# MinJunKang/DualPixelFace

Hardware: AMD Instinct MI355X
Metric: train samples/sec, StereoDPNet 1024x1536 DP pair (higher is better)
Workload: dtype f32

## Files before the change

### dualpixelface_amd/csrc/dcn_lean.hip

```cpp
#include "dcn_internal.h"
#include "conv_internal.h"

namespace {

typedef float f32x2 __attribute__((ext_vector_type(2)));

struct LeanP {
  int B, C, K, D, H, W;
  int Cpad, KT;
  long long P;
  int tilesY, tilesX;
  int nchunk;
};

__device__ __forceinline__ int lean_xcd_tile(int blk, int n) {
  const int q = n >> 3, r = n & 7, x = blk & 7, i = blk >> 3;
  return x * q + (x < r ? x : r) + i;
}

template <int CH_, int TY_, int TX_, int RYH_, int RXL_, int RXR_>
struct Geo {
  static constexpr int CH = CH_, NQ = CH_ / 4, TY = TY_, TX = TX_, RYH = RYH_, RXL = RXL_;
  static constexpr int NV = 4 * TY * TX;
  static constexpr int RY = TY + 2 + 2 * RYH;
  static constexpr int RX = (TX + 2 + RXL + RXR_ + 3) / 4 * 4;
  static constexpr int ZS = RY * RX * 16;
  static constexpr int PLANE = 4 * ZS;
  static constexpr int SQ = NV * 16;
  static constexpr int SBUF = NQ * SQ;
  static constexpr int LDS = NQ * PLANE + 2 * SBUF;
  static constexpr int NS = NV / 64;
  static_assert((1 + RXL) % 4 == 0 && TX % 16 == 0 && NV % 64 == 0, "aligned region origin / whole waves");
};

__device__ __forceinline__ int lane_pos32(int l) { return (int)((0x73261540u >> (4 * (l >> 2))) & 7u) * 4 + (l & 3); }

__device__ __forceinline__ f32x2 pk_mul_lo(f32x2 w, f32x2 v) {
  f32x2 r;
  asm("v_pk_mul_f32 %0, %1, %2 op_sel_hi:[0,1]" : "=v"(r) : "v"(w), "v"(v));
  return r;
}
__device__ __forceinline__ f32x2 pk_mul_hi(f32x2 w, f32x2 v) {
  f32x2 r;
  asm("v_pk_mul_f32 %0, %1, %2 op_sel:[1,0] op_sel_hi:[1,1]" : "=v"(r) : "v"(w), "v"(v));
  return r;
}
__device__ __forceinline__ void pk_fma_lo(f32x2& acc, f32x2 w, f32x2 v) {
  asm("v_pk_fma_f32 %0, %1, %2, %0 op_sel_hi:[0,1,1]" : "+v"(acc) : "v"(w), "v"(v));
}
__device__ __forceinline__ void pk_fma_hi(f32x2& acc, f32x2 w, f32x2 v) {
  asm("v_pk_fma_f32 %0, %1, %2, %0 op_sel:[1,0,0] op_sel_hi:[1,1,1]" : "+v"(acc) : "v"(w), "v"(v));
}

template <class G>
__device__ __forceinline__ void lean_stage(const LeanP& p, const float* __restrict__ xb, int c0, char* region, int ry0, int rx0, int tid,
                                           int nthreads) {
  constexpr int SR = G::RX / 4;
  const long long chan = p.P;
  const int units = p.D * G::RY * G::NQ * SR;
  for (int u = tid; u < units; u += nthreads) {
    const int seg = u % SR;
    const int it = u / SR;
    const int cg = it % G::NQ;
    const int row = it / G::NQ;
    const int lz = row / G::RY, ly = row - lz * G::RY;
    const int gy = ry0 + ly, gx = rx0 + 4 * seg;
    const bool ok = gy >= 0 && gy < p.H && gx >= 0 && gx < p.W;
    const float* src = xb + (long long)(c0 + 4 * cg) * chan + ((long long)lz * p.H + gy) * p.W + gx;
    f32x4 v[4];
#pragma unroll
    for (int q = 0; q < 4; ++q) v[q] = (ok && c0 + 4 * cg + q < p.C) ? *reinterpret_cast<const f32x4*>(src + q * chan) : f32x4{0.f, 0.f, 0.f, 0.f};
    char* dst = region + cg * G::PLANE + (row * G::RX + 4 * seg) * 16;
    *reinterpret_cast<f32x4*>(dst) = f32x4{v[0].x, v[1].x, v[2].x, v[3].x};
    *reinterpret_cast<f32x4*>(dst + 16) = f32x4{v[0].y, v[1].y, v[2].y, v[3].y};
    *reinterpret_cast<f32x4*>(dst + 32) = f32x4{v[0].z, v[1].z, v[2].z, v[3].z};
    *reinterpret_cast<f32x4*>(dst + 48) = f32x4{v[0].w, v[1].w, v[2].w, v[3].w};
  }
}

struct LeanTab {
  int a0, a1;
  f32x2 w00, w01, w10, w11;
  int d0, h0, w0;
  float ld, lh, lw;
  bool inreg;
  bool slow;
  f32x2 wz, wy, wx;
  f32x2 mz;
};

template <class G>
__device__ __forceinline__ LeanTab lean_tab(const LeanP& p, bool pvalid, int ry0, int rx0, float fd, float fh, float fw) {
  LeanTab t;
  const float d0f = floorf(fd), h0f = floorf(fh), w0f = floorf(fw);
  t.ld = fd - d0f; t.lh = fh - h0f; t.lw = fw - w0f;
  t.d0 = (int)d0f; t.h0 = (int)h0f; t.w0 = (int)w0f;
  const int ly = t.h0 - ry0, lx = t.w0 - rx0;
  t.inreg = (unsigned)ly < (unsigned)(G::RY - 1) && (unsigned)lx < (unsigned)(G::RX - 1);
  const bool valid = pvalid && fd > -1.f && fh > -1.f && fw > -1.f && fd < (float)p.D && fh < (float)p.H && fw < (float)p.W;
  const bool ok = t.inreg && valid;
  t.slow = valid && !t.inreg;
  const bool mz0 = (unsigned)t.d0 < (unsigned)p.D, mz1 = (unsigned)(t.d0 + 1) < (unsigned)p.D;
  f32x2 wz, wy, wx;
  wz.x = (ok && mz0) ? 1.f - t.ld : 0.f;
  wz.y = (ok && mz1) ? t.ld : 0.f;
  wy.x = 1.f - t.lh; wy.y = t.lh;
  wx.x = 1.f - t.lw; wx.y = t.lw;
  t.wz = wz; t.wy = wy; t.wx = wx;
  t.mz.x = (ok && mz0) ? 1.f : 0.f; t.mz.y = (ok && mz1) ? 1.f : 0.f;
  const int Dm1 = p.D - 1;
  const int iz0 = min(max(t.d0, 0), Dm1), iz1 = min(max(t.d0 + 1, 0), Dm1);
  const int cell = ok ? __mul24(__mul24(iz0, G::RY) + ly, G::RX) + lx : 0;
  t.a0 = cell * 16;
  t.a1 = t.a0 + __mul24(iz1 - iz0, G::ZS);
  const f32x2 zy0 = pk_mul_lo(wz, wy), zy1 = pk_mul_hi(wz, wy);
  t.w00 = pk_mul_lo(zy0, wx); t.w01 = pk_mul_hi(zy0, wx);
  t.w10 = pk_mul_lo(zy1, wx); t.w11 = pk_mul_hi(zy1, wx);
  return t;
}

#define LEAN_LOAD8(dst, q)                                                                        \
  dst[0] = *reinterpret_cast<const f32x4*>(r0 + (q) * G::PLANE);                                  \
  dst[1] = *reinterpret_cast<const f32x4*>(r0 + (q) * G::PLANE + 16);                             \
  dst[2] = *reinterpret_cast<const f32x4*>(r0 + (q) * G::PLANE + G::RX * 16);                     \
  dst[3] = *reinterpret_cast<const f32x4*>(r0 + (q) * G::PLANE + G::RX * 16 + 16);                \
  dst[4] = *reinterpret_cast<const f32x4*>(r1 + (q) * G::PLANE);                                  \
  dst[5] = *reinterpret_cast<const f32x4*>(r1 + (q) * G::PLANE + 16);                             \
  dst[6] = *reinterpret_cast<const f32x4*>(r1 + (q) * G::PLANE + G::RX * 16);                     \
  dst[7] = *reinterpret_cast<const f32x4*>(r1 + (q) * G::PLANE + G::RX * 16 + 16);

template <int CH>
__global__ void lean_repack_fwd1_kernel(const float* __restrict__ w, float* __restrict__ wl, int K, int C, int MT, int nchunk) {
  const int total = 27 * nchunk * MT * 512;
  for (int i = blockIdx.x * blockDim.x + threadIdx.x; i < total; i += gridDim.x * blockDim.x) {
    const int s = i & 7, lane = (i >> 3) & 63;
    int r = i >> 9;
    const int m = r % MT; r /= MT;
    const int chunk = r % nchunk;
    const int t = r / nchunk;
    const int k = 32 * m + (lane & 31), cl = 2 * s + (lane >> 5), c = chunk * CH + cl;
    wl[i] = (cl < CH && k < K && c < C) ? w[((long long)k * C + c) * 27 + t] : 0.f;
  }
}

template <class G, int MT>
__global__ __launch_bounds__(256, 2) void dcn_lean_fwd1_kernel(const float* __restrict__ x, const float* __restrict__ offset,
                                                            const float* __restrict__ wl, const float* __restrict__ bias,
                                                            float* __restrict__ out, LeanP p) {
  extern __shared__ __align__(16) char smem[];
  constexpr int CH = G::CH, NQ = G::NQ, KSTEPS = CH / 2, T = 27;
  static_assert(G::NV == 256, "four waves of 64 voxels");
  char* region = smem;
  const int tid = threadIdx.x, lane = tid & 63, l31 = lane & 31, hh = lane >> 5;
  const int wave_u = __builtin_amdgcn_readfirstlane(tid >> 6);
  int blk = lean_xcd_tile(blockIdx.x, gridDim.x);
  const int tx = blk % p.tilesX; blk /= p.tilesX;
  const int ty = blk % p.tilesY;
  const int b = blk / p.tilesY;
  const int y0 = ty * G::TY, x0 = tx * G::TX;
// ... 371 lines not shown
    tab1 = lean_tab<G>(p, pvalid, ry0, rx0, fd1, fh1, fw1);
  }
  int chunk = 0;
#pragma unroll 1
  for (int c0 = 0; c0 < p.C; c0 += CH, ++chunk) {
    __syncthreads();
    lean_stage<G>(p, xb, c0, region, ry0, rx0, tid, 256);
    load_a(0, chunk, aC);
    __syncthreads();
    sample_core();
    slow_fix(tab, nxt, c0);
    make_b(nxt, bH, bM, bL);
    tab = tab1;
#pragma unroll 1
    for (int t = 0; t < T - 1; ++t) {
      load_a(t + 1, chunk, aN);
      __builtin_amdgcn_sched_barrier(0);
      mfmas();
      sample_core();
      int u = t + 2;
      if (u >= T) u -= T;
      const LeanTab tabn = next_table(u);
#pragma unroll
      for (int i = 0; i < 4 * MT; ++i) {
        __builtin_amdgcn_sched_group_barrier(0x008, 1, 0);
        __builtin_amdgcn_sched_group_barrier(0x100, MT == 2 ? 2 : 4, 0);
        __builtin_amdgcn_sched_group_barrier(0x002, MT == 2 ? 2 : 4, 0);
      }
#pragma unroll
      for (int i = 0; i < 8 * MT; ++i) {
        __builtin_amdgcn_sched_group_barrier(0x008, 1, 0);
        __builtin_amdgcn_sched_group_barrier(0x002, MT == 2 ? 9 : 18, 0);
        __builtin_amdgcn_sched_group_barrier(0x100, MT == 2 ? 1 : 2, 0);
      }
      __builtin_amdgcn_sched_barrier(0);
      slow_fix(tab, nxt, c0);
      tab = tabn;
      make_b(nxt, bH, bM, bL);
#pragma unroll
      for (int m = 0; m < MT; ++m)
#pragma unroll
        for (int c = 0; c < 3; ++c) aC[m][c] = aN[m][c];
    }
    mfmas();
    tab1 = next_table(1);
  }
#pragma unroll
  for (int nt = 0; nt < 2; ++nt) {
    const int vo = wave_u * 64 + nt * 32 + lane_pos32(l31);
    const int qx = vo % G::TX, qy = (vo / G::TX) % G::TY, qz = vo / (G::TX * G::TY);
    const int gz = qz, gy = y0 + qy, gx = x0 + qx;
    const int q = l31 & 3;
    const bool o1 = (q & 1) != 0, o2 = (q & 2) != 0;
    const bool inb = gz < p.D && gy < p.H && gx < p.W;
    const long long pos = ((long long)gz * p.H + gy) * p.W + (gx - q);
#pragma unroll
    for (int m = 0; m < MT; ++m)
#pragma unroll
      for (int i = 0; i < 4; ++i) {
        float r0 = acc[m][nt][4 * i], r1 = acc[m][nt][4 * i + 1], r2 = acc[m][nt][4 * i + 2], r3 = acc[m][nt][4 * i + 3];
        {
          const float xa = o1 ? r0 : r1, ya = o1 ? r2 : r3;
          const float xs = __builtin_bit_cast(float, __builtin_amdgcn_mov_dpp(__builtin_bit_cast(int, xa), 0xB1, 0xf, 0xf, true));
          const float ys = __builtin_bit_cast(float, __builtin_amdgcn_mov_dpp(__builtin_bit_cast(int, ya), 0xB1, 0xf, 0xf, true));
          if (o1) { r0 = xs; r2 = ys; } else { r1 = xs; r3 = ys; }
        }
        {
          const float xa = o2 ? r0 : r2, ya = o2 ? r1 : r3;
          const float xs = __builtin_bit_cast(float, __builtin_amdgcn_mov_dpp(__builtin_bit_cast(int, xa), 0x4E, 0xf, 0xf, true));
          const float ys = __builtin_bit_cast(float, __builtin_amdgcn_mov_dpp(__builtin_bit_cast(int, ya), 0x4E, 0xf, 0xf, true));
          if (o2) { r0 = xs; r1 = ys; } else { r2 = xs; r3 = ys; }
        }
        const int k = m * 32 + 8 * i + 4 * hh + q;
        if (inb && k < p.K) {
          const float bv = bias ? bias[k] : 0.f;
          const f32x4 v = {r0 + bv, r1 + bv, r2 + bv, r3 + bv};
          *reinterpret_cast<f32x4*>(out + ((long long)b * p.K + k) * p.P + pos) = v;
        }
      }
  }
}

constexpr int LEAN_SS = 260;
constexpr int LEAN_NREP = DCN_WG_NREP;

template <class G>
struct BwdLds {
  static constexpr int GT = G::NQ * G::SQ;
  static constexpr int ST = G::CH * LEAN_SS * 4;
  static constexpr int OFF_G = G::NQ * G::PLANE;
  static constexpr int OFF_S = OFF_G + 2 * GT;
  static constexpr int LDS = OFF_S + 2 * ST;
  static_assert(G::NV == 256, "4 sampler waves + 4 matrix waves of 64 voxels");
};

typedef _Float16 lean_f16x8 __attribute__((ext_vector_type(8)));
typedef unsigned lean_u32x4 __attribute__((ext_vector_type(4)));
template <class G, bool GH>
__global__ __launch_bounds__(512) void dcn_lean_bwd_offset_kernel(const float* __restrict__ x, const float* __restrict__ offset,
                                                                  const float* __restrict__ wg ,
                                                                  const float* __restrict__ go, float* __restrict__ doff, float* __restrict__ dwtmp,
                                                                  LeanP p, int det) {
  extern __shared__ __align__(16) char smem[];
  constexpr int CH = G::CH, NQ = G::NQ, T = 27;
  typedef BwdLds<G> L;
  char* region = smem;
  const int tid = threadIdx.x, lane = tid & 63;
  const int wave_u = __builtin_amdgcn_readfirstlane(tid >> 6);
  int blk = lean_xcd_tile(blockIdx.x, gridDim.x);
  const int tx = blk % p.tilesX; blk /= p.tilesX;
  const int ty = blk % p.tilesY;
  const int b = blk / p.tilesY;
  const int y0 = ty * G::TY, x0 = tx * G::TX;
  const int ry0 = y0 - 1 - G::RYH, rx0 = x0 - 1 - G::RXL;
  const float* xb = x + (long long)b * p.C * p.P;
  const float* gob = go + (long long)b * p.K * p.P;
  const int NS = p.nchunk * T;
  if (wave_u < 4) {
    const int vox = wave_u * 64 + (lane & 32) + lane_pos32(lane & 31);
    const int px = vox % G::TX, py = (vox / G::TX) % G::TY, pz = vox / (G::TX * G::TY);
    const int zo = pz, yo = y0 + py, xo = x0 + px;
    const bool pvalid = zo < p.D && yo < p.H && xo < p.W;
    const long long ppos = pvalid ? ((long long)zo * p.H + yo) * p.W + xo : 0;
    const float* offp0 = offset + (long long)b * 3 * T * p.P + ppos;
    float* doffp0 = doff + (long long)b * 3 * T * p.P + ppos;
    const float zbf = (float)(zo - 1), ybf = (float)(yo - 1), xbf = (float)(xo - 1);
    const long long P3 = 3 * p.P;
    float od[3], oh[3], ow[3];
    LeanTab tab = lean_tab<G>(p, pvalid, ry0, rx0, zbf + offp0[0], ybf + offp0[p.P], xbf + offp0[2 * p.P]);
#pragma unroll
    for (int u = 1; u <= 3; ++u) { od[u % 3] = offp0[u * P3]; oh[u % 3] = offp0[u * P3 + p.P]; ow[u % 3] = offp0[u * P3 + 2 * p.P]; }
    lean_stage<G>(p, xb, 0, region, ry0, rx0, tid, 512);
    __syncthreads();
    int i = 0;
#pragma unroll 1
    for (int c0 = 0; c0 < p.C; c0 += CH) {
      if (c0 > 0) {
        lean_stage<G>(p, xb, c0, region, ry0, rx0, tid, 512);
        __syncthreads();
      }
#pragma unroll 1
      for (int g = 0; g < 9; ++g) {
        const int gn = g < 8 ? g + 1 : 0;
        const int ti = g / 3, tj = g - 3 * ti, tin = gn / 3, tjn = gn - 3 * tin;
        const float fz_same = zbf + (float)ti, fy_same = ybf + (float)tj, fz_next = zbf + (float)tin, fy_next = ybf + (float)tjn;
#pragma unroll
        for (int r = 0; r < 3; ++r, ++i) {
          const int t = 3 * g + r;
          const int sl = (r + 1) % 3;
          const float fdn = (r < 2 ? fz_same : fz_next) + od[sl], fhn = (r < 2 ? fy_same : fy_next) + oh[sl];
          const float fwn = (xbf + (float)((r + 1) % 3)) + ow[sl];
          {
            int u = t + 4;
            if (u >= T) u -= T;
            const float* np = offp0 + (long long)u * P3;
            od[sl] = np[0]; oh[sl] = np[p.P]; ow[sl] = np[2 * p.P];
          }
          const char* gt = smem + L::OFF_G + (i & 1) * L::GT + vox * 16;
          float* st = reinterpret_cast<float*>(smem + L::OFF_S + (i & 1) * L::ST);
          const char* r0 = region + tab.a0;
          const char* r1 = region + tab.a1;
          const f32x2 w00 = pk_mul_lo(pk_mul_lo(tab.wz, tab.wy), tab.wx), w01 = pk_mul_hi(pk_mul_lo(tab.wz, tab.wy), tab.wx);
          const f32x2 w10 = pk_mul_lo(pk_mul_hi(tab.wz, tab.wy), tab.wx), w11 = pk_mul_hi(pk_mul_hi(tab.wz, tab.wy), tab.wx);
          f32x4 cr[2][8], gq[2];
          LEAN_LOAD8(cr[0], 0)
          gq[0] = *reinterpret_cast<const f32x4*>(gt);
          LeanTab tabn = lean_tab<G>(p, pvalid, ry0, rx0, fdn, fhn, fwn);
          f32x2 dot[8];
#pragma unroll
          for (int q = 0; q < NQ; ++q) {
            if (q + 1 < NQ) {
              LEAN_LOAD8(cr[(q + 1) & 1], q + 1)
              gq[(q + 1) & 1] = *reinterpret_cast<const f32x4*>(gt + (q + 1) * G::SQ);
            }
            const f32x4* c = cr[q & 1];
            const f32x2 glo = gq[q & 1].xy, ghi = gq[q & 1].zw;
            f32x2 lo = pk_mul_lo(w00, c[0].xy), hi = pk_mul_lo(w00, c[0].zw);
            pk_fma_hi(lo, w00, c[1].xy); pk_fma_hi(hi, w00, c[1].zw);
            pk_fma_lo(lo, w01, c[2].xy); pk_fma_lo(hi, w01, c[2].zw);
            pk_fma_hi(lo, w01, c[3].xy); pk_fma_hi(hi, w01, c[3].zw);
            pk_fma_lo(lo, w10, c[4].xy); pk_fma_lo(hi, w10, c[4].zw);
            pk_fma_hi(lo, w10, c[5].xy); pk_fma_hi(hi, w10, c[5].zw);
            pk_fma_lo(lo, w11, c[6].xy); pk_fma_lo(hi, w11, c[6].zw);
            pk_fma_hi(lo, w11, c[7].xy); pk_fma_hi(hi, w11, c[7].zw);
            st[(4 * q + 0) * LEAN_SS + vox] = lo.x; st[(4 * q + 1) * LEAN_SS + vox] = lo.y;
            st[(4 * q + 2) * LEAN_SS + vox] = hi.x; st[(4 * q + 3) * LEAN_SS + vox] = hi.y;
#pragma unroll
            for (int j = 0; j < 8; ++j) {
              if (q == 0) dot[j] = glo * c[j].xy; else dot[j] = __builtin_elementwise_fma(glo, c[j].xy, dot[j]);
              dot[j] = __builtin_elementwise_fma(ghi, c[j].zw, dot[j]);
            }
          }
          float gd, gh, gw;
          {
            float d[8];
#pragma unroll
            for (int j = 0; j < 8; ++j) d[j] = dot[j].x + dot[j].y;
            const float wx0 = tab.wx.x, wx1 = tab.wx.y, wy0 = tab.wy.x, wy1 = tab.wy.y, wz0 = tab.wz.x, wz1 = tab.wz.y;
            const float A00 = fmaf(wx1, d[1], wx0 * d[0]), A01 = fmaf(wx1, d[3], wx0 * d[2]);
            const float A10 = fmaf(wx1, d[5], wx0 * d[4]), A11 = fmaf(wx1, d[7], wx0 * d[6]);
            const float E00 = fmaf(wy1, d[2], wy0 * d[0]), E01 = fmaf(wy1, d[3], wy0 * d[1]);
            const float E10 = fmaf(wy1, d[6], wy0 * d[4]), E11 = fmaf(wy1, d[7], wy0 * d[5]);
            const float B0 = fmaf(wy1, A01, wy0 * A00), B1 = fmaf(wy1, A11, wy0 * A10);
            gd = fmaf(tab.mz.y, B1, -tab.mz.x * B0);
            gh = fmaf(wz1, A11 - A10, wz0 * (A01 - A00));
            gw = fmaf(wz1, E11 - E10, wz0 * (E01 - E00));
          }
          unsigned long long slow = __ballot(tab.slow);
          while (slow) {
            const int Lq = __builtin_ctzll(slow);
            slow &= slow - 1;
            const int sd0 = __builtin_amdgcn_readlane(tab.d0, Lq), sh0 = __builtin_amdgcn_readlane(tab.h0, Lq), sw0 = __builtin_amdgcn_readlane(tab.w0, Lq);
            const float sld = __builtin_bit_cast(float, __builtin_amdgcn_readlane(__builtin_bit_cast(int, tab.ld), Lq));
            const float slh = __builtin_bit_cast(float, __builtin_amdgcn_readlane(__builtin_bit_cast(int, tab.lh), Lq));
            const float slw = __builtin_bit_cast(float, __builtin_amdgcn_readlane(__builtin_bit_cast(int, tab.lw), Lq));
            const int svox = __builtin_amdgcn_readlane(vox, Lq);
            const int ch = lane & 15, jd = lane >> 5, jh = (lane >> 4) & 1;
            const int dz = sd0 + jd, hy = sh0 + jh;
            const int cgl = c0 + ch;
            const bool rowin = ch < CH && cgl < p.C && (unsigned)dz < (unsigned)p.D && (unsigned)hy < (unsigned)p.H;
            const bool in0 = rowin && (unsigned)sw0 < (unsigned)p.W, in1 = rowin && (unsigned)(sw0 + 1) < (unsigned)p.W;
            const float* xr = xb + (long long)(cgl < p.C ? cgl : 0) * p.P + ((long long)(rowin ? dz : 0) * p.H + (rowin ? hy : 0)) * p.W;
            const float v0 = in0 ? xr[sw0] : 0.f, v1 = in1 ? xr[sw0 + 1] : 0.f;
            const float gch = ch < CH ? *reinterpret_cast<const float*>(smem + L::OFF_G + (i & 1) * L::GT + (ch >> 2) * G::SQ + svox * 16 + (ch & 3) * 4) : 0.f;
            const float wzj = jd ? sld : 1.f - sld, wyj = jh ? slh : 1.f - slh;
            float part = (wzj * wyj) * fmaf(slw, v1, (1.f - slw) * v0);
            part += __shfl_xor(part, 16, 64);
            part += __shfl_xor(part, 32, 64);
            if (lane < CH) st[lane * LEAN_SS + svox] = part;
            float e0 = gch * v0, e1 = gch * v1;
#pragma unroll
            for (int m = 1; m < 16; m <<= 1) { e0 += __shfl_xor(e0, m, 64); e1 += __shfl_xor(e1, m, 64); }
            const float ex = fmaf(slw, e1, (1.f - slw) * e0);
            float sgd = (jd ? 1.f : -1.f) * wyj * ex;
            float sgh = (jh ? 1.f : -1.f) * wzj * ex;
            float sgw = wzj * wyj * (e1 - e0);
            sgd += __shfl_xor(sgd, 16, 64); sgd += __shfl_xor(sgd, 32, 64);
            sgh += __shfl_xor(sgh, 16, 64); sgh += __shfl_xor(sgh, 32, 64);
            sgw += __shfl_xor(sgw, 16, 64); sgw += __shfl_xor(sgw, 32, 64);
            if (lane == Lq) { gd = sgd; gh = sgh; gw = sgw; }
          }
          if (pvalid) {
            float* dq = doffp0 + (long long)(3 * t) * p.P;
            if (c0 == 0) { dq[0] = gd; dq[p.P] = gh; dq[2 * p.P] = gw; }
            else { atomicAdd(dq, gd); atomicAdd(dq + p.P, gh); atomicAdd(dq + 2 * p.P, gw); }
          }
          tab = tabn;
          __syncthreads();
        }
      }
    }
  } else {
    const int mw = wave_u - 4, l15 = lane & 15, lg = lane >> 4;
    float bfrag[GH ? 1 : 4][16];
    lean_u32x4 bq[GH ? 4 : 1][2][2];
    int Egv[GH ? 4 : 1], Ew = DPF_H3_EMIN;
    if constexpr (GH) {
      Ew = __builtin_amdgcn_readfirstlane(reinterpret_cast<const int*>(wg)[27 * p.nchunk * 1024]);
#pragma unroll
      for (int s4 = 0; s4 < 4; ++s4) {
        const int vox = mw * 64 + s4 * 16 + l15;
        const int px = vox % G::TX, py = (vox / G::TX) % G::TY, pz = vox / (G::TX * G::TY);
        const bool ok = pz < p.D && y0 + py < p.H && x0 + px < p.W;
        const long long gpos = ok ? ((long long)pz * p.H + y0 + py) * p.W + x0 + px : 0;
        float gv[16];
        float mxg = 0.f;
#pragma unroll
        for (int mf = 0; mf < 2; ++mf)
#pragma unroll
          for (int i = 0; i < 8; ++i) {
            const int k = 32 * mf + 8 * lg + i;
            gv[8 * mf + i] = (ok && k < p.K) ? gob[(long long)k * p.P + gpos] : 0.f;
            mxg = __builtin_fmaxf(mxg, __builtin_fabsf(gv[8 * mf + i]));
          }
        mxg = __builtin_fmaxf(mxg, __shfl_xor(mxg, 16, 64));
        mxg = __builtin_fmaxf(mxg, __shfl_xor(mxg, 32, 64));
        int e = (int)(__builtin_bit_cast(unsigned, mxg) >> 23);
        e = e < DPF_H3_EMIN ? DPF_H3_EMIN : (e > 254 ? 254 : e);
        Egv[s4] = e;
        const float scg = dpf_h3_scale(e);
#pragma unroll
        for (int mf = 0; mf < 2; ++mf)
#pragma unroll
          for (int i = 0; i < 4; ++i) {
            unsigned h, l;
            dpf_split_pair_h(gv[8 * mf + 2 * i] * scg, gv[8 * mf + 2 * i + 1] * scg, h, l);
            bq[s4][mf][0][i] = h; bq[s4][mf][1][i] = l;
          }
      }
    } else {
#pragma unroll
      for (int s4 = 0; s4 < 4; ++s4) {
        const int vox = mw * 64 + s4 * 16 + l15;
        const int px = vox % G::TX, py = (vox / G::TX) % G::TY, pz = vox / (G::TX * G::TY);
        const bool ok = pz < p.D && y0 + py < p.H && x0 + px < p.W;
        const long long gpos = ok ? ((long long)pz * p.H + y0 + py) * p.W + x0 + px : 0;
#pragma unroll
        for (int ks = 0; ks < 16; ++ks) {
          const int k = 4 * ks + lg;
          bfrag[s4][ks] = (ok && k < p.K) ? gob[(long long)k * p.P + gpos] : 0.f;
        }
      }
    }
    float wfrag[64];
    {
      const int kk = 16 * mw + l15;
#pragma unroll
      for (int ks = 0; ks < 64; ++ks) {
        const int vox = 16 * (ks >> 2) + 4 * lg + (ks & 3);
        const int px = vox % G::TX, py = (vox / G::TX) % G::TY, pz = vox / (G::TX * G::TY);
        const bool ok = kk < p.K && pz < p.D && y0 + py < p.H && x0 + px < p.W;
        wfrag[ks] = ok ? gob[(long long)kk * p.P + ((long long)pz * p.H + y0 + py) * p.W + x0 + px] : 0.f;
      }
    }
    float* rep = det ? dwtmp : dwtmp + (long long)(blockIdx.x % LEAN_NREP) * T * p.nchunk * 64 * 16;
    long long* rep_shadow = det ? reinterpret_cast<long long*>(dwtmp) : nullptr;
    const int brow = (l15 < CH ? l15 : CH - 1) * LEAN_SS + 4 * lg;
    const unsigned wlane = (unsigned)lane * 64u;
    auto gcol = [&](int j) {
      const int chunk = j / T, t = j - chunk * T;
      const char* wb = reinterpret_cast<const char*>(wg) + (long long)(t * p.nchunk + chunk) * 4096;
      char* dst = smem + L::OFF_G + (j & 1) * L::GT + lg * G::SQ + (mw * 64 + l15) * 16;
      f32x4 a4[4];
      lean_u32x4 aq[2][2];
      if constexpr (GH) {
#pragma unroll
        for (int u = 0; u < 4; ++u) aq[u >> 1][u & 1] = *reinterpret_cast<const lean_u32x4*>(wb + u * 1024 + lane * 16);
      } else {
#pragma unroll
        for (int u = 0; u < 4; ++u) a4[u] = *reinterpret_cast<const f32x4*>(wb + wlane + 16 * u);
      }
#pragma unroll
      for (int sp2 = 0; sp2 < 2; ++sp2) {
        f32x4 acc[2] = {f32x4{0.f, 0.f, 0.f, 0.f}, f32x4{0.f, 0.f, 0.f, 0.f}};
        if constexpr (GH) {
          constexpr int ca[3] = {1, 0, 0}, cb[3] = {0, 1, 0};
#pragma unroll
          for (int i = 0; i < 3; ++i)
#pragma unroll
            for (int mf = 0; mf < 2; ++mf)
#pragma unroll
              for (int u = 0; u < 2; ++u)
                acc[u] = __builtin_amdgcn_mfma_f32_16x16x32_f16(__builtin_bit_cast(lean_f16x8, aq[mf][ca[i]]),
                                                                 __builtin_bit_cast(lean_f16x8, bq[2 * sp2 + u][mf][cb[i]]), acc[u], 0, 0, 0);
#pragma unroll
          for (int u = 0; u < 2; ++u)
#pragma unroll
            for (int r = 0; r < 4; ++r) acc[u][r] = __builtin_ldexpf(acc[u][r], Egv[2 * sp2 + u] + Ew - 282);
        } else {
#pragma unroll
          for (int ks = 0; ks < 16; ++ks)
#pragma unroll
            for (int u = 0; u < 2; ++u) acc[u] = __builtin_amdgcn_mfma_f32_16x16x4f32(a4[ks >> 2][ks & 3], bfrag[2 * sp2 + u][ks], acc[u], 0, 0, 0);
        }
        if (lg < NQ) {
          *reinterpret_cast<f32x4*>(dst + (2 * sp2) * 256) = acc[0];
          *reinterpret_cast<f32x4*>(dst + (2 * sp2 + 1) * 256) = acc[1];
        }
      }
    };
    gcol(0);
    lean_stage<G>(p, xb, 0, region, ry0, rx0, tid, 512);
    __syncthreads();
#pragma unroll 1
    for (int i = 0; i <= NS; ++i) {
      if (i + 1 < NS) gcol(i + 1);
      if (i >= 1) {
        const int j = i - 1, cs = j / T, ts = j - cs * T;
        const float* src = reinterpret_cast<const float*>(smem + L::OFF_S + (j & 1) * L::ST) + brow;
        f32x4 wacc[4] = {f32x4{0.f, 0.f, 0.f, 0.f}, f32x4{0.f, 0.f, 0.f, 0.f}, f32x4{0.f, 0.f, 0.f, 0.f}, f32x4{0.f, 0.f, 0.f, 0.f}};
#pragma unroll
        for (int qq = 0; qq < 16; ++qq) {
          const f32x4 bv = *reinterpret_cast<const f32x4*>(src + 16 * qq);
          wacc[0] = __builtin_amdgcn_mfma_f32_16x16x4f32(wfrag[4 * qq + 0], bv.x, wacc[0], 0, 0, 0);
          wacc[1] = __builtin_amdgcn_mfma_f32_16x16x4f32(wfrag[4 * qq + 1], bv.y, wacc[1], 0, 0, 0);
          wacc[2] = __builtin_amdgcn_mfma_f32_16x16x4f32(wfrag[4 * qq + 2], bv.z, wacc[2], 0, 0, 0);
          wacc[3] = __builtin_amdgcn_mfma_f32_16x16x4f32(wfrag[4 * qq + 3], bv.w, wacc[3], 0, 0, 0);
        }
        if (l15 < CH && cs * CH + l15 < p.C) {
          float* dst = rep + ((long long)(ts * p.nchunk + cs) * 64 + 16 * mw + 4 * lg) * 16 + l15;
#pragma unroll
          for (int r = 0; r < 4; ++r)
            if (16 * mw + 4 * lg + r < p.K) dcn_acc_add(rep, rep_shadow, &dst[r * 16], (wacc[0][r] + wacc[1][r]) + (wacc[2][r] + wacc[3][r]));
        }
      }
      if (i < NS) {
        __syncthreads();
        if (i + 1 < NS && (i + 1) % T == 0) {
          lean_stage<G>(p, xb, ((i + 1) / T) * CH, region, ry0, rx0, tid, 512);
          __syncthreads();
        }
      }
    }
  }
}

__global__ void lean_repack_gcol_kernel(const float* __restrict__ w, float* __restrict__ wg, int K, int C, int CH, int nchunk) {
  const int total = 27 * nchunk * 1024;
  for (int i = blockIdx.x * blockDim.x + threadIdx.x; i < total; i += gridDim.x * blockDim.x) {
    const int ks = i & 15, lane = (i >> 4) & 63;
    const int r = i >> 10;
    const int chunk = r % nchunk, t = r / nchunk;
    const int k = 4 * ks + (lane >> 4), l15 = lane & 15, c = chunk * CH + l15;
    wg[i] = (k < K && l15 < CH && c < C) ? w[((long long)k * C + c) * 27 + t] : 0.f;
  }
}

__global__ void lean_repack_gcol_h_kernel(const float* __restrict__ w, unsigned short* __restrict__ wgh, int K, int C, int CH, int nchunk) {
  __shared__ int s_e[16];
  float m = 0.f;
  const int nw = K * C * 27;
  for (int i = threadIdx.x; i < nw; i += blockDim.x) m = __builtin_fmaxf(m, __builtin_fabsf(w[i]));
  const int e = dpf_wave_max_exp(__builtin_bit_cast(unsigned, m));
  if ((threadIdx.x & 63) == 0) s_e[threadIdx.x >> 6] = e;
  __syncthreads();
  int E = DPF_H3_EMIN;
  for (int i = 0; i < (int)(blockDim.x >> 6); ++i) E = s_e[i] > E ? s_e[i] : E;
  E = E > 254 ? 254 : E;
  const float sc = dpf_h3_scale(E);
  const int total = 27 * nchunk * 2048;
  if (blockIdx.x == 0 && threadIdx.x == 0) reinterpret_cast<int*>(wgh)[total / 2] = E;
  for (int i = blockIdx.x * blockDim.x + threadIdx.x; i < total; i += gridDim.x * blockDim.x) {
    const int idx = i & 7, lane = (i >> 3) & 63, comp = (i >> 9) & 1, mf = (i >> 10) & 1;
    const int r = i >> 11;
    const int chunk = r % nchunk, t = r / nchunk;
    const int k = 32 * mf + 8 * (lane >> 4) + idx, l15 = lane & 15, c = chunk * CH + l15;
    const float v = (k < K && l15 < CH && c < C) ? w[((long long)k * C + c) * 27 + t] * sc : 0.f;
    unsigned h, l;
    dpf_split_pair_h(v, 0.f, h, l);
    wgh[i] = (unsigned short)((comp ? l : h) & 0xffffu);
  }
}

template <class G, bool SIX>
int lean_launch_fwd(const float* x, const float* offset, const float* weight, const float* bias, float* out, float* ws, LeanP p, hipStream_t st) {
  p.tilesY = dpf_div_up(p.H, G::TY);
  p.tilesX = dpf_div_up(p.W, G::TX);
  const long long blocks = (long long)p.B * p.tilesY * p.tilesX;
  if (blocks >= 0x7fffffffLL) return DPF_ERR_UNSUPPORTED;
  const int MT = p.KT / 32;
  constexpr int LDS = G::NQ * G::PLANE;
  const dim3 grid_w(dpf_ew_grid(27LL * p.nchunk * MT * 512)), grid((unsigned)blocks), block(256);
  int rc;
  if constexpr (SIX) {
    unsigned short* wl = reinterpret_cast<unsigned short*>(ws);
    hipLaunchKernelGGL((lean_repack_fwd6_kernel<G::CH>), grid_w, block, 0, st, weight, wl, p.K, p.C, MT, p.nchunk);
    rc = dcn_launch(MT == 1 ? dcn_lean_fwd6_kernel<G, 1> : dcn_lean_fwd6_kernel<G, 2>, grid, block, LDS, st, x, offset, wl, bias, out, p);
  } else {
    hipLaunchKernelGGL((lean_repack_fwd1_kernel<G::CH>), grid_w, block, 0, st, weight, ws, p.K, p.C, MT, p.nchunk);
    rc = dcn_launch(MT == 1 ? dcn_lean_fwd1_kernel<G, 1> : dcn_lean_fwd1_kernel<G, 2>, grid, block, LDS, st, x, offset, ws, bias, out, p);
  }
  return rc != DPF_OK ? rc : dpf_check_launch();
}

typedef Geo<16, 4, 16, 3, 3, 3> G16c;
typedef Geo<12, 4, 16, 5, 7, 4> G12c;
typedef Geo<12, 4, 16, 5, 3, 3> G12d;

typedef Geo<16, 4, 16, 4, 3, 3> B16;
typedef Geo<12, 4, 16, 5, 7, 4> B12;

template <class G>
int lean_launch_bwd_offset(const float* x, const float* offset, const float* weight, const float* go, float* doff, float* dwtmp, float* ws, LeanP p,
                           hipStream_t st, int det) {
  p.tilesY = dpf_div_up(p.H, G::TY);
  p.tilesX = dpf_div_up(p.W, G::TX);
  const long long blocks = (long long)p.B * p.tilesY * p.tilesX;
  if (blocks >= 0x7fffffffLL) return DPF_ERR_UNSUPPORTED;
  const dim3 grid((unsigned)blocks), block(512);
  int rc;
  if (dcn_env().gcol16 && dpf_conv_f32_x9() == 2) {
    hipLaunchKernelGGL(lean_repack_gcol_h_kernel, dim3(16), dim3(1024), 0, st, weight, reinterpret_cast<unsigned short*>(ws), p.K, p.C, G::CH, p.nchunk);
    rc = dcn_launch(dcn_lean_bwd_offset_kernel<G, true>, grid, block, BwdLds<G>::LDS + 64, st, x, offset, ws, go, doff, dwtmp, p, det);
  } else {
    hipLaunchKernelGGL(lean_repack_gcol_kernel, dim3(dpf_ew_grid(27LL * p.nchunk * 1024)), dim3(256), 0, st, weight, ws, p.K, p.C, G::CH, p.nchunk);
    rc = dcn_launch(dcn_lean_bwd_offset_kernel<G, false>, grid, block, BwdLds<G>::LDS, st, x, offset, ws, go, doff, dwtmp, p, det);
  }
  return rc != DPF_OK ? rc : dpf_check_launch();
}

bool lean_params(LeanP& p, const float* x, int B, int C, int D, int H, int W, int K) {
  if (D > 4 || D < 1 || (W & 3) || K > 64 || (reinterpret_cast<uintptr_t>(x) & 15)) return false;
  if ((long long)D * H * W >= 0x7fffffffLL / 4) return false;
  const int CH = dcn_chunk(C);
  p = LeanP{};
  p.B = B; p.C = C; p.K = K; p.D = D; p.H = H; p.W = W;
  p.Cpad = (C + CH - 1) / CH * CH;
  p.nchunk = p.Cpad / CH;
  p.KT = 32 * ((K + 31) / 32);
  p.P = (long long)D * H * W;
  return true;
}

}

long long dcn_lean_workspace_floats(int C, int K) {
  const int CH = dcn_chunk(C);
  const long long nchunk = (C + CH - 1) / CH;
  const long long fwd = 27LL * nchunk * ((K + 31) / 32) * 768;
  const long long bwd = 27LL * nchunk * 1024 + 16;
  return fwd > bwd ? fwd : bwd;
}

int dcn_lean_forward(const float* x, const float* offset, const float* weight, const float* bias, float* out, float* ws, int B, int C, int D, int H,
                     int W, int K, hipStream_t st) {
  const DcnEnv& env = dcn_env();
  LeanP p;
  if (!env.lean || (reinterpret_cast<uintptr_t>(out) & 15) || !lean_params(p, x, B, C, D, H, W, K)) return DPF_ERR_UNSUPPORTED;
  const bool ch16 = dcn_chunk(C) == 16;
  if (env.fwd6 && dpf_conv_f32_x9()) {
    if (ch16) return lean_launch_fwd<G16c, true>(x, offset, weight, bias, out, ws, p, st);
    return lean_launch_fwd<G12d, true>(x, offset, weight, bias, out, ws, p, st);
  }
  if (ch16) return lean_launch_fwd<G16c, false>(x, offset, weight, bias, out, ws, p, st);
  if (env.lean_wide12) return lean_launch_fwd<G12c, false>(x, offset, weight, bias, out, ws, p, st);
  return lean_launch_fwd<G12d, false>(x, offset, weight, bias, out, ws, p, st);
}

int dcn_lean_bwd_offset(const float* x, const float* offset, const float* weight, const float* go, float* doff, float* dwtmp, float* ws, int B, int C,
                        int D, int H, int W, int K, hipStream_t st, int det) {
  const int lean = dcn_env().lean;
  LeanP p;
  if (!lean || (lean & 4) || !lean_params(p, x, B, C, D, H, W, K)) return DPF_ERR_UNSUPPORTED;
  if (dcn_chunk(C) == 16) return lean_launch_bwd_offset<B16>(x, offset, weight, go, doff, dwtmp, ws, p, st, det);
  return lean_launch_bwd_offset<B12>(x, offset, weight, go, doff, dwtmp, ws, p, st, det);
}
```

Measured before the change: 27.33.

## Use split-f16 MFMA with per-channel exponent scaling for DCN weight-grad GEMM

In the gcol16 path of the lean DCN backward-offset kernel, the weight-gradient GEMM now runs on f16x32 MFMA instead of f32x4 MFMA. Operands are split into hi/lo f16 pairs, three products are accumulated, and the result is rescaled with ldexp. Staging tracks per-channel max exponents via LDS atomics so sampled values can be scaled into f16 range, with an f32 fallback for overflowing entries. The aim is to cut MFMA issue cost and LDS footprint, at the price of extra split and exponent bookkeeping and a small precision risk.

```diff
diff --git a/dualpixelface_amd/csrc/dcn_lean.hip b/dualpixelface_amd/csrc/dcn_lean.hip
--- a/dualpixelface_amd/csrc/dcn_lean.hip
+++ b/dualpixelface_amd/csrc/dcn_lean.hip
@@ -52,9 +52,9 @@
   asm("v_pk_fma_f32 %0, %1, %2, %0 op_sel:[1,0,0] op_sel_hi:[1,1,1]" : "+v"(acc) : "v"(w), "v"(v));
 }
 
-template <class G>
+template <class G, bool EXP = false>
 __device__ __forceinline__ void lean_stage(const LeanP& p, const float* __restrict__ xb, int c0, char* region, int ry0, int rx0, int tid,
-                                           int nthreads) {
+                                           int nthreads, int* exps = nullptr) {
   constexpr int SR = G::RX / 4;
   const long long chan = p.P;
   const int units = p.D * G::RY * G::NQ * SR;
@@ -75,6 +75,15 @@
     *reinterpret_cast<f32x4*>(dst + 16) = f32x4{v[0].y, v[1].y, v[2].y, v[3].y};
     *reinterpret_cast<f32x4*>(dst + 32) = f32x4{v[0].z, v[1].z, v[2].z, v[3].z};
     *reinterpret_cast<f32x4*>(dst + 48) = f32x4{v[0].w, v[1].w, v[2].w, v[3].w};
+    if constexpr (EXP) {
+#pragma unroll
+      for (int q = 0; q < 4; ++q) {
+        const float m = __builtin_fmaxf(__builtin_fmaxf(__builtin_fabsf(v[q].x), __builtin_fabsf(v[q].y)),
+                                        __builtin_fmaxf(__builtin_fabsf(v[q].z), __builtin_fabsf(v[q].w)));
+        const int e = (int)(__builtin_bit_cast(unsigned, m) >> 23);
+        if (e > exps[4 * cg + q]) atomicMax(&exps[4 * cg + q], e);
+      }
+    }
   }
 }
 
@@ -612,31 +621,40 @@
 }
 
 constexpr int LEAN_SS = 260;
+constexpr int LEAN_SH = 264;
 constexpr int LEAN_NREP = DCN_WG_NREP;
 
-template <class G>
+template <class G, bool WH>
 struct BwdLds {
   static constexpr int GT = G::NQ * G::SQ;
-  static constexpr int ST = G::CH * LEAN_SS * 4;
+  static constexpr int SP = G::CH * LEAN_SH * 2;
+  static constexpr int ST = WH ? 2 * SP : G::CH * LEAN_SS * 4;
   static constexpr int OFF_G = G::NQ * G::PLANE;
   static constexpr int OFF_S = OFF_G + 2 * GT;
-  static constexpr int LDS = OFF_S + 2 * ST;
+  static constexpr int OFF_E = OFF_S + 2 * ST;
+  static constexpr int LDS = OFF_E + (WH ? 2 * 16 * 4 : 0);
+  static_assert(LDS <= 160 * 1024 && OFF_E % 16 == 0, "one workgroup per CU");
   static_assert(G::NV == 256, "4 sampler waves + 4 matrix waves of 64 voxels");
 };
 
 typedef _Float16 lean_f16x8 __attribute__((ext_vector_type(8)));
 typedef unsigned lean_u32x4 __attribute__((ext_vector_type(4)));
-template <class G, bool GH>
+template <class G, bool GH, bool WH>
 __global__ __launch_bounds__(512) void dcn_lean_bwd_offset_kernel(const float* __restrict__ x, const float* __restrict__ offset,
                                                                   const float* __restrict__ wg ,
                                                                   const float* __restrict__ go, float* __restrict__ doff, float* __restrict__ dwtmp,
                                                                   LeanP p, int det) {
   extern __shared__ __align__(16) char smem[];
   constexpr int CH = G::CH, NQ = G::NQ, T = 27;
-  typedef BwdLds<G> L;
+  typedef BwdLds<G, WH> L;
   char* region = smem;
+  int* exps = reinterpret_cast<int*>(smem + L::OFF_E);
   const int tid = threadIdx.x, lane = tid & 63;
   const int wave_u = __builtin_amdgcn_readfirstlane(tid >> 6);
+  if constexpr (WH) {
+    if (tid < 32) exps[tid] = DPF_H3_EMIN;
+    __syncthreads();
+  }
   int blk = lean_xcd_tile(blockIdx.x, gridDim.x);
   const int tx = blk % p.tilesX; blk /= p.tilesX;
   const int ty = blk % p.tilesY;
@@ -646,6 +664,8 @@
   const float* xb = x + (long long)b * p.C * p.P;
   const float* gob = go + (long long)b * p.K * p.P;
   const int NS = p.nchunk * T;
+  float* rep = det ? dwtmp : dwtmp + (long long)(blockIdx.x % LEAN_NREP) * T * p.nchunk * 64 * 16;
+  long long* rep_shadow = det ? reinterpret_cast<long long*>(dwtmp) : nullptr;
   if (wave_u < 4) {
     const int vox = wave_u * 64 + (lane & 32) + lane_pos32(lane & 31);
     const int px = vox % G::TX, py = (vox / G::TX) % G::TY, pz = vox / (G::TX * G::TY);
@@ -660,14 +680,23 @@
     LeanTab tab = lean_tab<G>(p, pvalid, ry0, rx0, zbf + offp0[0], ybf + offp0[p.P], xbf + offp0[2 * p.P]);
 #pragma unroll
     for (int u = 1; u <= 3; ++u) { od[u % 3] = offp0[u * P3]; oh[u % 3] = offp0[u * P3 + p.P]; ow[u % 3] = offp0[u * P3 + 2 * p.P]; }
-    lean_stage<G>(p, xb, 0, region, ry0, rx0, tid, 512);
+    lean_stage<G, WH>(p, xb, 0, region, ry0, rx0, tid, 512, exps);
     __syncthreads();
     int i = 0;
 #pragma unroll 1
-    for (int c0 = 0; c0 < p.C; c0 += CH) {
+    for (int c0 = 0, chunk = 0; c0 < p.C; c0 += CH, ++chunk) {
       if (c0 > 0) {
-        lean_stage<G>(p, xb, c0, region, ry0, rx0, tid, 512);
+        lean_stage<G, WH>(p, xb, c0, region, ry0, rx0, tid, 512, exps + (chunk & 1) * 16);
         __syncthreads();
+      }
+      const int* cexp = exps + (chunk & 1) * 16;
+      float ssc[WH ? CH : 1];
+      if constexpr (WH) {
+#pragma unroll
+        for (int c = 0; c < CH; ++c) {
+          const int e = cexp[c];
+          ssc[c] = dpf_h3_scale(e > 254 ? 254 : e);
+        }
       }
 #pragma unroll 1
       for (int g = 0; g < 9; ++g) {
@@ -688,6 +717,8 @@
           }
           const char* gt = smem + L::OFF_G + (i & 1) * L::GT + vox * 16;
           float* st = reinterpret_cast<float*>(smem + L::OFF_S + (i & 1) * L::ST);
+          unsigned short* sth = reinterpret_cast<unsigned short*>(st);
+          unsigned short* stl = sth + CH * LEAN_SH;
           const char* r0 = region + tab.a0;
           const char* r1 = region + tab.a1;
           const f32x2 w00 = pk_mul_lo(pk_mul_lo(tab.wz, tab.wy), tab.wx), w01 = pk_mul_hi(pk_mul_lo(tab.wz, tab.wy), tab.wx);
@@ -713,8 +744,18 @@
             pk_fma_hi(lo, w10, c[5].xy); pk_fma_hi(hi, w10, c[5].zw);
             pk_fma_lo(lo, w11, c[6].xy); pk_fma_lo(hi, w11, c[6].zw);
             pk_fma_hi(lo, w11, c[7].xy); pk_fma_hi(hi, w11, c[7].zw);
-            st[(4 * q + 0) * LEAN_SS + vox] = lo.x; st[(4 * q + 1) * LEAN_SS + vox] = lo.y;
-            st[(4 * q + 2) * LEAN_SS + vox] = hi.x; st[(4 * q + 3) * LEAN_SS + vox] = hi.y;
+            if constexpr (WH) {
+              unsigned h0, l0, h1, l1;
+              dpf_split_pair_h(lo.x * ssc[4 * q], lo.y * ssc[4 * q + 1], h0, l0);
+              dpf_split_pair_h(hi.x * ssc[4 * q + 2], hi.y * ssc[4 * q + 3], h1, l1);
+              sth[(4 * q + 0) * LEAN_SH + vox] = (unsigned short)h0; sth[(4 * q + 1) * LEAN_SH + vox] = (unsigned short)(h0 >> 16);
+              sth[(4 * q + 2) * LEAN_SH + vox] = (unsigned short)h1; sth[(4 * q + 3) * LEAN_SH + vox] = (unsigned short)(h1 >> 16);
+              stl[(4 * q + 0) * LEAN_SH + vox] = (unsigned short)l0; stl[(4 * q + 1) * LEAN_SH + vox] = (unsigned short)(l0 >> 16);
+              stl[(4 * q + 2) * LEAN_SH + vox] = (unsigned short)l1; stl[(4 * q + 3) * LEAN_SH + vox] = (unsigned short)(l1 >> 16);
+            } else {
+              st[(4 * q + 0) * LEAN_SS + vox] = lo.x; st[(4 * q + 1) * LEAN_SS + vox] = lo.y;
+              st[(4 * q + 2) * LEAN_SS + vox] = hi.x; st[(4 * q + 3) * LEAN_SS + vox] = hi.y;
+            }
 #pragma unroll
             for (int j = 0; j < 8; ++j) {
               if (q == 0) dot[j] = glo * c[j].xy; else dot[j] = __builtin_elementwise_fma(glo, c[j].xy, dot[j]);
@@ -757,7 +798,24 @@
             float part = (wzj * wyj) * fmaf(slw, v1, (1.f - slw) * v0);
             part += __shfl_xor(part, 16, 64);
             part += __shfl_xor(part, 32, 64);
-            if (lane < CH) st[lane * LEAN_SS + svox] = part;
+            if constexpr (WH) {
+              if (lane < CH) {
+                const int e = cexp[lane];
+                float sv = part * dpf_h3_scale(e > 254 ? 254 : e);
+                if (!(__builtin_fabsf(sv) < 32768.f)) {
+                  const int spx = svox % G::TX, spy = (svox / G::TX) % G::TY, spz = svox / (G::TX * G::TY);
+                  const float* gp = gob + ((long long)spz * p.H + y0 + spy) * p.W + x0 + spx;
+                  float* dq = rep + ((long long)(t * p.nchunk + chunk) * 64) * 16 + lane;
+                  for (int k = 0; k < p.K; ++k) dcn_acc_add(rep, rep_shadow, dq + k * 16, gp[(long long)k * p.P] * part);
+                  sv = 0.f;
+                }
+                unsigned h, l;
+                dpf_split_pair_h(sv, 0.f, h, l);
+                sth[lane * LEAN_SH + svox] = (unsigned short)h; stl[lane * LEAN_SH + svox] = (unsigned short)l;
+              }
+            } else {
+              if (lane < CH) st[lane * LEAN_SS + svox] = part;
+            }
             float e0 = gch * v0, e1 = gch * v1;
 #pragma unroll
             for (int m = 1; m < 16; m <<= 1) { e0 += __shfl_xor(e0, m, 64); e1 += __shfl_xor(e1, m, 64); }
@@ -832,20 +890,49 @@
         }
       }
     }
-    float wfrag[64];
+    float wfrag[WH ? 1 : 64];
+    lean_u32x4 wah[WH ? 8 : 1], wal[WH ? 8 : 1];
+    int Erow[4] = {0, 0, 0, 0};
+    const int wbase = 128 * (lg & 1) + 64 * (lg >> 1);
     {
       const int kk = 16 * mw + l15;
-#pragma unroll
-      for (int ks = 0; ks < 64; ++ks) {
-        const int vox = 16 * (ks >> 2) + 4 * lg + (ks & 3);
-        const int px = vox % G::TX, py = (vox / G::TX) % G::TY, pz = vox / (G::TX * G::TY);
-        const bool ok = kk < p.K && pz < p.D && y0 + py < p.H && x0 + px < p.W;
-        wfrag[ks] = ok ? gob[(long long)kk * p.P + ((long long)pz * p.H + y0 + py) * p.W + x0 + px] : 0.f;
-      }
-    }
-    float* rep = det ? dwtmp : dwtmp + (long long)(blockIdx.x % LEAN_NREP) * T * p.nchunk * 64 * 16;
-    long long* rep_shadow = det ? reinterpret_cast<long long*>(dwtmp) : nullptr;
-    const int brow = (l15 < CH ? l15 : CH - 1) * LEAN_SS + 4 * lg;
+      if constexpr (WH) {
+        float mxg = 0.f, gv[64];
+#pragma unroll
+        for (int j = 0; j < 64; ++j) {
+          const int vox = wbase + j;
+          const int px = vox % G::TX, py = (vox / G::TX) % G::TY, pz = vox / (G::TX * G::TY);
+          const bool ok = kk < p.K && pz < p.D && y0 + py < p.H && x0 + px < p.W;
+          gv[j] = ok ? gob[(long long)kk * p.P + ((long long)pz * p.H + y0 + py) * p.W + x0 + px] : 0.f;
+          mxg = __builtin_fmaxf(mxg, __builtin_fabsf(gv[j]));
+        }
+        mxg = __builtin_fmaxf(mxg, __shfl_xor(mxg, 16, 64));
+        mxg = __builtin_fmaxf(mxg, __shfl_xor(mxg, 32, 64));
+        int e = (int)(__builtin_bit_cast(unsigned, mxg) >> 23);
+        e = e < DPF_H3_EMIN ? DPF_H3_EMIN : (e > 254 ? 254 : e);
+        const float scg = dpf_h3_scale(e);
+#pragma unroll
+        for (int ks = 0; ks < 8; ++ks)
+#pragma unroll
+          for (int i = 0; i < 4; ++i) {
+            unsigned h, l;
+            dpf_split_pair_h(gv[8 * ks + 2 * i] * scg, gv[8 * ks + 2 * i + 1] * scg, h, l);
+            wah[ks][i] = h; wal[ks][i] = l;
+          }
+#pragma unroll
+        for (int r = 0; r < 4; ++r) Erow[r] = __shfl(e, 4 * lg + r, 64) - 282;
+      } else {
+#pragma unroll
+        for (int ks = 0; ks < 64; ++ks) {
+          const int vox = 16 * (ks >> 2) + 4 * lg + (ks & 3);
+          const int px = vox % G::TX, py = (vox / G::TX) % G::TY, pz = vox / (G::TX * G::TY);
+          const bool ok = kk < p.K && pz < p.D && y0 + py < p.H && x0 + px < p.W;
+          wfrag[ks] = ok ? gob[(long long)kk * p.P + ((long long)pz * p.H + y0 + py) * p.W + x0 + px] : 0.f;
+        }
+      }
+    }
+    const int ccol = l15 < CH ? l15 : CH - 1;
+    const int brow = WH ? (ccol * LEAN_SH + wbase) * 2  : ccol * LEAN_SS + 4 * lg ;
     const unsigned wlane = (unsigned)lane * 64u;
     auto gcol = [&](int j) {
       const int chunk = j / T, t = j - chunk * T;
@@ -890,34 +977,56 @@
       }
     };
     gcol(0);
-    lean_stage<G>(p, xb, 0, region, ry0, rx0, tid, 512);
+    lean_stage<G, WH>(p, xb, 0, region, ry0, rx0, tid, 512, exps);
     __syncthreads();
 #pragma unroll 1
     for (int i = 0; i <= NS; ++i) {
       if (i + 1 < NS) gcol(i + 1);
       if (i >= 1) {
         const int j = i - 1, cs = j / T, ts = j - cs * T;
-        const float* src = reinterpret_cast<const float*>(smem + L::OFF_S + (j & 1) * L::ST) + brow;
         f32x4 wacc[4] = {f32x4{0.f, 0.f, 0.f, 0.f}, f32x4{0.f, 0.f, 0.f, 0.f}, f32x4{0.f, 0.f, 0.f, 0.f}, f32x4{0.f, 0.f, 0.f, 0.f}};
-#pragma unroll
-        for (int qq = 0; qq < 16; ++qq) {
-          const f32x4 bv = *reinterpret_cast<const f32x4*>(src + 16 * qq);
-          wacc[0] = __builtin_amdgcn_mfma_f32_16x16x4f32(wfrag[4 * qq + 0], bv.x, wacc[0], 0, 0, 0);
-          wacc[1] = __builtin_amdgcn_mfma_f32_16x16x4f32(wfrag[4 * qq + 1], bv.y, wacc[1], 0, 0, 0);
-          wacc[2] = __builtin_amdgcn_mfma_f32_16x16x4f32(wfrag[4 * qq + 2], bv.z, wacc[2], 0, 0, 0);
-          wacc[3] = __builtin_amdgcn_mfma_f32_16x16x4f32(wfrag[4 * qq + 3], bv.w, wacc[3], 0, 0, 0);
+        float wsum[4];
+        if constexpr (WH) {
+          const char* src = smem + L::OFF_S + (j & 1) * L::ST + brow;
+          const int ec = exps[(cs & 1) * 16 + ccol];
+          const int Ecol = ec > 254 ? 254 : ec;
+#pragma unroll
+          for (int ks = 0; ks < 8; ++ks) {
+            const lean_f16x8 bh = __builtin_bit_cast(lean_f16x8, *reinterpret_cast<const lean_u32x4*>(src + 16 * ks));
+            const lean_f16x8 bl = __builtin_bit_cast(lean_f16x8, *reinterpret_cast<const lean_u32x4*>(src + L::SP + 16 * ks));
+            wacc[0] = __builtin_amdgcn_mfma_f32_16x16x32_f16(__builtin_bit_cast(lean_f16x8, wal[ks]), bh, wacc[0], 0, 0, 0);
+            wacc[1] = __builtin_amdgcn_mfma_f32_16x16x32_f16(__builtin_bit_cast(lean_f16x8, wah[ks]), bl, wacc[1], 0, 0, 0);
+            wacc[2] = __builtin_amdgcn_mfma_f32_16x16x32_f16(__builtin_bit_cast(lean_f16x8, wah[ks]), bh, wacc[2], 0, 0, 0);
+          }
+#pragma unroll
+          for (int r = 0; r < 4; ++r) wsum[r] = __builtin_ldexpf((wacc[0][r] + wacc[1][r]) + wacc[2][r], Erow[r] + Ecol);
+        } else {
+          const float* src = reinterpret_cast<const float*>(smem + L::OFF_S + (j & 1) * L::ST) + brow;
+#pragma unroll
+          for (int qq = 0; qq < 16; ++qq) {
+            const f32x4 bv = *reinterpret_cast<const f32x4*>(src + 16 * qq);
+            wacc[0] = __builtin_amdgcn_mfma_f32_16x16x4f32(wfrag[4 * qq + 0], bv.x, wacc[0], 0, 0, 0);
+            wacc[1] = __builtin_amdgcn_mfma_f32_16x16x4f32(wfrag[4 * qq + 1], bv.y, wacc[1], 0, 0, 0);
+            wacc[2] = __builtin_amdgcn_mfma_f32_16x16x4f32(wfrag[4 * qq + 2], bv.z, wacc[2], 0, 0, 0);
+            wacc[3] = __builtin_amdgcn_mfma_f32_16x16x4f32(wfrag[4 * qq + 3], bv.w, wacc[3], 0, 0, 0);
+          }
+#pragma unroll
+          for (int r = 0; r < 4; ++r) wsum[r] = (wacc[0][r] + wacc[1][r]) + (wacc[2][r] + wacc[3][r]);
         }
         if (l15 < CH && cs * CH + l15 < p.C) {
           float* dst = rep + ((long long)(ts * p.nchunk + cs) * 64 + 16 * mw + 4 * lg) * 16 + l15;
 #pragma unroll
           for (int r = 0; r < 4; ++r)
-            if (16 * mw + 4 * lg + r < p.K) dcn_acc_add(rep, rep_shadow, &dst[r * 16], (wacc[0][r] + wacc[1][r]) + (wacc[2][r] + wacc[3][r]));
+            if (16 * mw + 4 * lg + r < p.K) dcn_acc_add(rep, rep_shadow, &dst[r * 16], wsum[r]);
         }
       }
       if (i < NS) {
         __syncthreads();
+        if constexpr (WH) {
+          if (i % T == 1 && mw == 0 && lane < 16) exps[((i / T + 1) & 1) * 16 + lane] = DPF_H3_EMIN;
+        }
         if (i + 1 < NS && (i + 1) % T == 0) {
-          lean_stage<G>(p, xb, ((i + 1) / T) * CH, region, ry0, rx0, tid, 512);
+          lean_stage<G, WH>(p, xb, ((i + 1) / T) * CH, region, ry0, rx0, tid, 512, exps + (((i + 1) / T) & 1) * 16);
           __syncthreads();
         }
       }
@@ -1001,10 +1110,10 @@
   int rc;
   if (dcn_env().gcol16 && dpf_conv_f32_x9() == 2) {
     hipLaunchKernelGGL(lean_repack_gcol_h_kernel, dim3(16), dim3(1024), 0, st, weight, reinterpret_cast<unsigned short*>(ws), p.K, p.C, G::CH, p.nchunk);
-    rc = dcn_launch(dcn_lean_bwd_offset_kernel<G, true>, grid, block, BwdLds<G>::LDS + 64, st, x, offset, ws, go, doff, dwtmp, p, det);
+    rc = dcn_launch(dcn_lean_bwd_offset_kernel<G, true, true>, grid, block, BwdLds<G, true>::LDS, st, x, offset, ws, go, doff, dwtmp, p, det);
   } else {
     hipLaunchKernelGGL(lean_repack_gcol_kernel, dim3(dpf_ew_grid(27LL * p.nchunk * 1024)), dim3(256), 0, st, weight, ws, p.K, p.C, G::CH, p.nchunk);
-    rc = dcn_launch(dcn_lean_bwd_offset_kernel<G, false>, grid, block, BwdLds<G>::LDS, st, x, offset, ws, go, doff, dwtmp, p, det);
+    rc = dcn_launch(dcn_lean_bwd_offset_kernel<G, false, false>, grid, block, BwdLds<G, false>::LDS, st, x, offset, ws, go, doff, dwtmp, p, det);
   }
   return rc != DPF_OK ? rc : dpf_check_launch();
 }
```

Result: faster. 27.75, median of 6 (+1.5%).
